# robotic-vision-lab/CropNeRF-A-Neural-Radiance-Field-Based-Framework

Measured on AMD Instinct MI355X. Metric: ray_samples_per_sec, higher is better.
Workload: dtype f32 (matrix products: bf16 hi+lo operand split, f32 accumulate); 1 GPU; plant_1-shaped synthetic scene (P-rand), 800x800, 192 samples/ray, 65536-ray batch, mode M-uniform, fused cn_render_rays, eval (no jitter); rays_per_batch=65536, samples_per_ray=192, mode=uniform, matrix_precision=split_bf16 (FruitNerfModelConfig default; exact fp32: secondary.exact_fp32_ms)

## Files before the change

### cropnerf-a-neural-radiance-field-based-framework_amd/csrc/cn_common.hpp

```cpp
#pragma once

#include <hip/hip_runtime.h>

#include <cstdarg>
#include <cstdio>
#include <cstring>
#include <mutex>
#include <type_traits>

#include "../../include/cropnerf_hip.h"

#define CN_WAVE 64

namespace cn {

void set_error(const char* fmt, ...);

inline int check_launch(const char* what) {
  hipError_t e = hipGetLastError();
  if (e != hipSuccess) {
    set_error("%s: %s", what, hipGetErrorString(e));
    return CN_ERR_LAUNCH;
  }
  return CN_OK;
}

#define CN_REQUIRE(cond, code, ...) \
  do {                              \
    if (!(cond)) {                  \
      cn::set_error(__VA_ARGS__);   \
      return (code);                \
    }                               \
  } while (0)

inline hipStream_t as_stream(cn_stream_t s) { return reinterpret_cast<hipStream_t>(s); }

// ... 35 lines not shown
#define CN_P2 805459861u

struct Lvl {
  unsigned off, mask, m1, m2;
  float scale;
};

struct GridDev {
  const void* table;
  int num_levels;
  int half;
  float pos_offset;
  unsigned off[CN_MAX_LEVELS], mask[CN_MAX_LEVELS], m1[CN_MAX_LEVELS], m2[CN_MAX_LEVELS];
  float scale[CN_MAX_LEVELS];
  __host__ __device__ __forceinline__ Lvl level(int l) const {
    Lvl v;
    v.off = off[l];
    v.mask = mask[l];
    v.m1 = m1[l];
    v.m2 = m2[l];
    v.scale = scale[l];
    return v;
  }
  __host__ __device__ __forceinline__ const float* table_f32() const { return static_cast<const float*>(table); }
};

inline GridDev make_grid_dev(const cn_grid& g) {
  GridDev d;
  d.table = g.table;
  d.num_levels = g.num_levels;
  d.half = g.table_dtype == CN_TABLE_F16;
  d.pos_offset = g.layout == CN_GRID_TCNN ? 0.5f : 0.f;
  const unsigned T = 1u << g.log2_table_size;
  for (int i = 0; i < CN_MAX_LEVELS; ++i) {
    const bool live = i < g.num_levels;
    d.scale[i] = live ? g.scalings[i] : 0.f;
    const int b = (live && g.layout == CN_GRID_TCNN) ? g.level_bits[i] : 0;
    d.off[i] = !live ? 0u : (g.layout == CN_GRID_TCNN ? g.level_offset[i] : (unsigned)i * T);
    d.m1[i] = b ? 1u << b : CN_P1;
    d.m2[i] = b ? 1u << (2 * b) : CN_P2;
    d.mask[i] = b ? (1u << (3 * b)) - 1u : T - 1u;
  }
  return d;
}

inline int check_grid(const cn_grid& g, bool need_f32, const char* who) {
  CN_REQUIRE(g.table, CN_ERR_INVALID, "%s: null hash table", who);
  CN_REQUIRE(g.num_levels >= 1 && g.num_levels <= CN_MAX_LEVELS, CN_ERR_UNSUPPORTED, "%s: %d grid levels", who,
             g.num_levels);
  CN_REQUIRE(g.layout == CN_GRID_TORCH || g.layout == CN_GRID_TCNN, CN_ERR_INVALID, "%s: grid layout %d", who, g.layout);
  CN_REQUIRE(g.table_dtype == CN_TABLE_F32 || g.table_dtype == CN_TABLE_F16, CN_ERR_INVALID, "%s: table dtype %d", who,
             g.table_dtype);
  CN_REQUIRE(!need_f32 || g.table_dtype == CN_TABLE_F32, CN_ERR_UNSUPPORTED,
             "%s: needs an fp32 hash table (half tables are inference-only)", who);
  CN_REQUIRE(g.log2_table_size >= 1 && g.log2_table_size <= 24, CN_ERR_UNSUPPORTED, "%s: log2 table size %d", who,
             g.log2_table_size);
  unsigned long long entries = (unsigned long long)g.num_levels << g.log2_table_size;
  if (g.layout == CN_GRID_TCNN) {
    entries = 0;
    for (int l = 0; l < g.num_levels; ++l) {
      const int b = g.level_bits[l];
      CN_REQUIRE(b <= 9, CN_ERR_UNSUPPORTED, "%s: dense level %d with %d bits per axis", who, l, b);
      CN_REQUIRE(g.level_offset[l] % 2 == 0, CN_ERR_INVALID, "%s: level %d starts at the odd entry %u", who, l,
                 g.level_offset[l]);
      const unsigned long long end = (unsigned long long)g.level_offset[l] + (b ? 1ull << (3 * b) : 1ull << g.log2_table_size);
      if (end > entries) entries = end;
    }
  }
  CN_REQUIRE(entries * 8ull <= (1ull << 31), CN_ERR_UNSUPPORTED, "%s: hash table larger than 2 GiB", who);
  const uintptr_t align = g.table_dtype == CN_TABLE_F16 ? 7u : 15u;
  CN_REQUIRE((reinterpret_cast<uintptr_t>(g.table) & align) == 0, CN_ERR_INVALID,
             "%s: the hash table must be %u-byte aligned", who, (unsigned)align + 1u);
  return CN_OK;
}
// ... 61 lines not shown
      const float coef = 2.f * inv * inv * (inv - 1.f) * s;
      gx *= k;
      gy *= k;
      gz *= k;
      if (axv >= ayv && axv >= azv) gx += x < 0.f ? -coef : coef;
      else if (ayv >= azv) gy += y < 0.f ? -coef : coef;
      else gz += z < 0.f ? -coef : coef;
    }
  } else {
    gx *= sc.inv_extent[0] * sel;
    gy *= sc.inv_extent[1] * sel;
    gz *= sc.inv_extent[2] * sel;
  }
}

typedef const float __attribute__((address_space(4)))* cfloat_ptr;
__device__ __forceinline__ cfloat_ptr as_const(const float* p) { return (cfloat_ptr)(unsigned long long)p; }

template <bool HALF = false>
__device__ __forceinline__ float2 hash_gather(const void* __restrict__ table, unsigned entry) {
  if constexpr (HALF) {
    typedef _Float16 h2 __attribute__((ext_vector_type(2)));
    const h2 v = *reinterpret_cast<const h2*>(reinterpret_cast<const char*>(table) + (size_t)(entry << 2));
    return make_float2((float)v.x, (float)v.y);
  } else {
    return *reinterpret_cast<const float2*>(reinterpret_cast<const char*>(table) + (size_t)(entry << 3));
  }
}

struct Cell {
  float ox, oy, oz;
  unsigned hx0, hx1, hy0, hy1, hz0, hz1;
};
template <bool OFFSET = true>
__device__ __forceinline__ Cell hash_cell(const Lvl& lv, float pos_offset, float px, float py, float pz) {
  const float sx = OFFSET ? fmaf(px, lv.scale, pos_offset) : px * lv.scale;
  const float sy = OFFSET ? fmaf(py, lv.scale, pos_offset) : py * lv.scale;
  const float sz = OFFSET ? fmaf(pz, lv.scale, pos_offset) : pz * lv.scale;
  const float fx = floorf(sx), fy = floorf(sy), fz = floorf(sz);
  Cell c;
  c.ox = sx - fx;
  c.oy = sy - fy;
  c.oz = sz - fz;
  const unsigned ix = (unsigned)(int)fx, iy = (unsigned)(int)fy, iz = (unsigned)(int)fz;
  c.hx0 = ix;
  c.hx1 = ix + 1u;
  c.hy0 = __umul24(iy, lv.m1);
  c.hy1 = c.hy0 + lv.m1;
  c.hz0 = __umul24(iz, lv.m2);
  c.hz1 = c.hz0 + lv.m2;
  return c;
}

template <bool HALF = false>
__device__ __forceinline__ float2 hash_level(const void* __restrict__ table, const Lvl& lv, float pos_offset, float px,
                                             float py, float pz) {
  const Cell k = hash_cell(lv, pos_offset, px, py, pz);
  const float ox = k.ox, oy = k.oy, oz = k.oz;
  float2 ccc = hash_gather<HALF>(table, ((k.hx1 ^ k.hy1 ^ k.hz1) & lv.mask) + lv.off);
  float2 cfc = hash_gather<HALF>(table, ((k.hx1 ^ k.hy0 ^ k.hz1) & lv.mask) + lv.off);
  float2 ffc = hash_gather<HALF>(table, ((k.hx0 ^ k.hy0 ^ k.hz1) & lv.mask) + lv.off);
  float2 fcc = hash_gather<HALF>(table, ((k.hx0 ^ k.hy1 ^ k.hz1) & lv.mask) + lv.off);
  float2 ccf = hash_gather<HALF>(table, ((k.hx1 ^ k.hy1 ^ k.hz0) & lv.mask) + lv.off);
  float2 cff = hash_gather<HALF>(table, ((k.hx1 ^ k.hy0 ^ k.hz0) & lv.mask) + lv.off);
  float2 fff = hash_gather<HALF>(table, ((k.hx0 ^ k.hy0 ^ k.hz0) & lv.mask) + lv.off);
  float2 fcf = hash_gather<HALF>(table, ((k.hx0 ^ k.hy1 ^ k.hz0) & lv.mask) + lv.off);
  float mx = 1.f - ox, my = 1.f - oy, mz = 1.f - oz;
  typedef float v2f __attribute__((ext_vector_type(2)));
  auto V = [](float2 t) {
    v2f v;
    v.x = t.x;
    v.y = t.y;
    return v;
  };
  const v2f f03 = V(ccc) * ox + V(fcc) * mx, f12 = V(cfc) * ox + V(ffc) * mx;
  const v2f f56 = V(cff) * ox + V(fff) * mx, f47 = V(ccf) * ox + V(fcf) * mx;
  const v2f a = f03 * oy + f12 * my, b = f47 * oy + f56 * my;
// ... 17 lines not shown
  float2 ccf = hash_gather<HALF>(table, ((k.hx1 ^ k.hy1 ^ k.hz0) & lv.mask) + lv.off);
  float2 cff = hash_gather<HALF>(table, ((k.hx1 ^ k.hy0 ^ k.hz0) & lv.mask) + lv.off);
  float2 fff = hash_gather<HALF>(table, ((k.hx0 ^ k.hy0 ^ k.hz0) & lv.mask) + lv.off);
  float2 fcf = hash_gather<HALF>(table, ((k.hx0 ^ k.hy1 ^ k.hz0) & lv.mask) + lv.off);
  const float mx = 1.f - ox, my = 1.f - oy, mz = 1.f - oz;
  auto V = [](float2 t) {
    v2f_t v;
    v.x = t.x;
    v.y = t.y;
    return v;
  };
  const v2f_t f03 = V(ccc) * ox + V(fcc) * mx, f12 = V(cfc) * ox + V(ffc) * mx;
  const v2f_t f56 = V(cff) * ox + V(fff) * mx, f47 = V(ccf) * ox + V(fcf) * mx;
  const v2f_t a = f03 * oy + f12 * my, b = f47 * oy + f56 * my;
  const v2f_t rv = a * oz + b * mz;
  const v2f_t d03 = V(ccc) - V(fcc), d12 = V(cfc) - V(ffc), d56 = V(cff) - V(fff), d47 = V(ccf) - V(fcf);
  jx = ((d03 * oy + d12 * my) * oz + (d47 * oy + d56 * my) * mz) * lv.scale;
  jy = ((f03 - f12) * oz + (f47 - f56) * mz) * lv.scale;
  jz = (a - b) * lv.scale;
  float2 r;
  r.x = rv.x;
  r.y = rv.y;
  return r;
}

template <bool HALF>
struct XpLoads {
  typedef float f4 __attribute__((ext_vector_type(4)));
  typedef _Float16 h4 __attribute__((ext_vector_type(4)));
  typedef _Float16 h2 __attribute__((ext_vector_type(2)));
  typename std::conditional<HALF, h4, f4>::type pr[4];
  typename std::conditional<HALF, h2, float2>::type up[4];
  unsigned bits;
  float ox, oy, oz;
};
template <bool HALF = false>
__device__ __forceinline__ XpLoads<HALF> hash_level_xpair_issue(const void* __restrict__ table, const Lvl& lv, float pos_offset,
                                                                float px, float py, float pz) {
  const Cell k = hash_cell(lv, pos_offset, px, py, pz);
  const char* base = reinterpret_cast<const char*>(table);
  const unsigned pair_mask = lv.mask & ~1u;
  const unsigned hyz[4] = {k.hy0 ^ k.hz0, k.hy1 ^ k.hz0, k.hy0 ^ k.hz1, k.hy1 ^ k.hz1};
  const bool odd = (k.hx0 & 1u) != 0u;
  XpLoads<HALF> L;
  L.bits = odd ? 16u : 0u;
  L.ox = k.ox;
  L.oy = k.oy;
  L.oz = k.oz;
#pragma unroll
  for (int r = 0; r < 4; ++r) {
    const unsigned x = k.hx0 ^ hyz[r];
    L.bits |= (x & 1u) << r;
    const unsigned e = (x & pair_mask) + lv.off;
    if constexpr (HALF) L.pr[r] = *reinterpret_cast<const typename XpLoads<HALF>::h4*>(base + (size_t)(e << 2));
    else L.pr[r] = *reinterpret_cast<const typename XpLoads<HALF>::f4*>(base + (size_t)(e << 3));
  }
#pragma unroll
  for (int r = 0; r < 4; ++r) {
    if constexpr (HALF) L.up[r] = typename XpLoads<HALF>::h2{(_Float16)0.f, (_Float16)0.f};
    else L.up[r] = make_float2(0.f, 0.f);
  }
  if (odd) {
#pragma unroll
    for (int r = 0; r < 4; ++r) {
      const unsigned e = ((k.hx1 ^ hyz[r]) & lv.mask) + lv.off;
      if constexpr (HALF) L.up[r] = *reinterpret_cast<const typename XpLoads<HALF>::h2*>(base + (size_t)(e << 2));
      else L.up[r] = *reinterpret_cast<const float2*>(base + (size_t)(e << 3));
    }
  }
  return L;
}
template <bool HALF = false>
__device__ __forceinline__ float2 hash_level_xpair_blend(const XpLoads<HALF>& L) {
  const bool odd = (L.bits & 16u) != 0u;
  typedef float v2f __attribute__((ext_vector_type(2)));
  const float ox = L.ox, oy = L.oy, oz = L.oz;
  const float mx = 1.f - ox, my = 1.f - oy, mz = 1.f - oz;
  const float oxe = odd ? 0.f : ox;
  v2f row[4];
#pragma unroll
  for (int r = 0; r < 4; ++r) {
    const bool second = ((L.bits >> r) & 1u) != 0u;
    const float wa = second ? oxe : mx, wb = second ? mx : oxe;
    v2f a, b, u;
    a.x = (float)L.pr[r].x;
    a.y = (float)L.pr[r].y;
    b.x = (float)L.pr[r].z;
    b.y = (float)L.pr[r].w;
    u.x = (float)L.up[r].x;
    u.y = (float)L.up[r].y;
    row[r] = u * ox + (b * wb + a * wa);
  }
  const v2f a2 = row[3] * oy + row[2] * my, b2 = row[1] * oy + row[0] * my;
  const v2f rv = a2 * oz + b2 * mz;
  float2 r;
  r.x = rv.x;
  r.y = rv.y;
  asm volatile("" : "+v"(r.x), "+v"(r.y));
  return r;
}
template <bool HALF = false>
__device__ __forceinline__ float2 hash_level_xpair(const void* __restrict__ table, const Lvl& lv, float pos_offset, float px,
                                                   float py, float pz) {
  return hash_level_xpair_blend<HALF>(hash_level_xpair_issue<HALF>(table, lv, pos_offset, px, py, pz));
}

__device__ __forceinline__ Lvl lane_level(const GridDev& g, int l) {
  Lvl v = g.level(0);
#pragma unroll
  for (int k = 1; k < CN_MAX_LEVELS; ++k) {
    const Lvl w = g.level(k);
    v.off = l == k ? w.off : v.off;
    v.mask = l == k ? w.mask : v.mask;
    v.m1 = l == k ? w.m1 : v.m1;
    v.m2 = l == k ? w.m2 : v.m2;
    v.scale = l == k ? w.scale : v.scale;
  }
  return v;
}

constexpr int LVL_REC_FLOATS = 16 + 64;
__device__ __forceinline__ void lds_level_fill(float* rec, const GridDev& g, int tid) {
  if (tid < CN_MAX_LEVELS) {
    const Lvl v = lane_level(g, tid);
// ... 29 lines not shown
  const Cell k = hash_cell<OFFSET>(lv, pos_offset, px, py, pz);
  const float ox = k.ox, oy = k.oy, oz = k.oz;
  float2 ccc = hash_gather<HALF>(table, ((k.hx1 ^ k.hy1 ^ k.hz1) & lv.mask) + lv.off);
  float2 cfc = hash_gather<HALF>(table, ((k.hx1 ^ k.hy0 ^ k.hz1) & lv.mask) + lv.off);
  float2 ffc = hash_gather<HALF>(table, ((k.hx0 ^ k.hy0 ^ k.hz1) & lv.mask) + lv.off);
  float2 fcc = hash_gather<HALF>(table, ((k.hx0 ^ k.hy1 ^ k.hz1) & lv.mask) + lv.off);
  float2 ccf = hash_gather<HALF>(table, ((k.hx1 ^ k.hy1 ^ k.hz0) & lv.mask) + lv.off);
  float2 cff = hash_gather<HALF>(table, ((k.hx1 ^ k.hy0 ^ k.hz0) & lv.mask) + lv.off);
  float2 fff = hash_gather<HALF>(table, ((k.hx0 ^ k.hy0 ^ k.hz0) & lv.mask) + lv.off);
  float2 fcf = hash_gather<HALF>(table, ((k.hx0 ^ k.hy1 ^ k.hz0) & lv.mask) + lv.off);
  float mx = 1.f - ox, my = 1.f - oy, mz = 1.f - oz;
  float2 r;
  {
    float f03 = ccc.x * ox + fcc.x * mx, f12 = cfc.x * ox + ffc.x * mx;
    float f56 = cff.x * ox + fff.x * mx, f47 = ccf.x * ox + fcf.x * mx;
    float a = f03 * oy + f12 * my, b = f47 * oy + f56 * my;
    r.x = a * oz + b * mz;
  }
  {
    float f03 = ccc.y * ox + fcc.y * mx, f12 = cfc.y * ox + ffc.y * mx;
    float f56 = cff.y * ox + fff.y * mx, f47 = ccf.y * ox + fcf.y * mx;
    float a = f03 * oy + f12 * my, b = f47 * oy + f56 * my;
    r.y = a * oz + b * mz;
  }
  return r;
}

typedef _Float16 f16x2 __attribute__((ext_vector_type(2)));
typedef unsigned u32x2p __attribute__((ext_vector_type(2)));
struct PkLoads {
  u32x2p pr[4];
  unsigned up[4];
  unsigned bits;
  unsigned wxy, wzz;
};
template <bool OFFSET = true>
__device__ __forceinline__ PkLoads hash_level_pk_issue(const void* __restrict__ table, const Lvl& lv, float pos_offset, float px,
                                                       float py, float pz) {
  const Cell k = hash_cell<OFFSET>(lv, pos_offset, px, py, pz);
  const char* base = reinterpret_cast<const char*>(table);
  const unsigned pair_mask = lv.mask & ~1u;
  const unsigned hyz[4] = {k.hy0 ^ k.hz0, k.hy1 ^ k.hz0, k.hy0 ^ k.hz1, k.hy1 ^ k.hz1};
  PkLoads L;
  {
    const _Float16 hx = (_Float16)k.ox, hy = (_Float16)k.oy, hz = (_Float16)k.oz;
    const f16x2 xy = {hx, hy}, zz = {hz, hz};
    L.wxy = __builtin_bit_cast(unsigned, xy);
    L.wzz = __builtin_bit_cast(unsigned, zz);
  }
  const bool odd = (k.hx0 & 1u) != 0u;
  L.bits = odd ? 16u : 0u;
#pragma unroll
  for (int r = 0; r < 4; ++r) {
    const unsigned x = k.hx0 ^ hyz[r];
    L.bits |= (x & 1u) << r;
    L.pr[r] = *reinterpret_cast<const u32x2p*>(base + (size_t)(((x & pair_mask) + lv.off) << 2));
    L.up[r] = 0u;
  }
#if !defined(CN_ABLATE_X1)
  if (odd) {
#pragma unroll
    for (int r = 0; r < 4; ++r) {
      L.up[r] = *reinterpret_cast<const unsigned*>(base + (size_t)((((k.hx1 ^ hyz[r]) & lv.mask) + lv.off) << 2));
    }
  }
#endif
  return L;
}
__device__ __forceinline__ unsigned hash_level_pk_blend(const PkLoads& L) {
  const bool odd = (L.bits & 16u) != 0u;
  f16x2 lo[4], hi[4];
#pragma unroll
  for (int r = 0; r < 4; ++r) {
    const bool second = (L.bits & (1u << r)) != 0u;
    const unsigned a = L.pr[r].x, b = L.pr[r].y;
    lo[r] = __builtin_bit_cast(f16x2, second ? b : a);
    const unsigned upv = L.up[r];
    hi[r] = __builtin_bit_cast(f16x2, odd ? upv : (second ? a : b));
  }
  const f16x2 wxy = __builtin_bit_cast(f16x2, L.wxy), wz = __builtin_bit_cast(f16x2, L.wzz);
  const f16x2 wx = {wxy.x, wxy.x}, wy = {wxy.y, wxy.y};
  const f16x2 xff = lo[0] + (hi[0] - lo[0]) * wx, xcf = lo[1] + (hi[1] - lo[1]) * wx;
  const f16x2 xfc = lo[2] + (hi[2] - lo[2]) * wx, xcc = lo[3] + (hi[3] - lo[3]) * wx;
  const f16x2 yf = xff + (xcf - xff) * wy, yc = xfc + (xcc - xfc) * wy;
  const f16x2 r = yf + (yc - yf) * wz;
  return __builtin_bit_cast(unsigned, r);
}
__device__ __forceinline__ unsigned pk_pin(unsigned v) {
  asm volatile("" : "+v"(v));
  return v;
}
template <bool OFFSET = true>
__device__ __forceinline__ unsigned hash_level_pk(const void* __restrict__ table, const Lvl& lv, float pos_offset, float px,
                                                  float py, float pz) {
  return hash_level_pk_blend(hash_level_pk_issue<OFFSET>(table, lv, pos_offset, px, py, pz));
}


__device__ __forceinline__ float linspace01(int i, int steps) {
  float step = 1.f / (float)(steps - 1);
  int half = steps / 2;
  return i < half ? step * (float)i : 1.f - step * (float)(steps - i - 1);
}

__device__ __forceinline__ float spacing_fn(int mode, float x) {
  if (mode == CN_SPACING_PIECEWISE) return x < 1.f ? x / 2.f : 1.f - 1.f / (2.f * x);
  return x;
}
__device__ __forceinline__ float spacing_fn_inv(int mode, float x) {
  if (mode == CN_SPACING_PIECEWISE) return x < 0.5f ? 2.f * x : 1.f / (2.f - 2.f * x);
  return x;
}
__device__ __forceinline__ float spacing_to_euclid(int mode, float x, float s_near, float s_far) {
  return spacing_fn_inv(mode, x * s_far + (1.f - x) * s_near);
}

__device__ __forceinline__ void sh_deg4(float x, float y, float z, float* c) {
  float xx = x * x, yy = y * y, zz = z * z;
  c[0] = 0.28209479177387814f;
  c[1] = 0.4886025119029199f * y;
  c[2] = 0.4886025119029199f * z;
  c[3] = 0.4886025119029199f * x;
  c[4] = 1.0925484305920792f * x * y;
  c[5] = 1.0925484305920792f * y * z;
  c[6] = 0.9461746957575601f * zz - 0.31539156525251999f;
  c[7] = 1.0925484305920792f * x * z;
  c[8] = 0.5462742152960396f * (xx - yy);
  c[9] = 0.5900435899266435f * y * (3.f * xx - yy);
  c[10] = 2.890611442640554f * x * y * z;
  c[11] = 0.4570457994644658f * y * (5.f * zz - 1.f);
  c[12] = 0.3731763325901154f * z * (5.f * zz - 3.f);
  c[13] = 0.4570457994644658f * x * (5.f * zz - 1.f);
  c[14] = 1.445305721320277f * z * (xx - yy);
  c[15] = 0.5900435899266435f * x * (xx - 3.f * yy);
}

// ... 9 lines not shown
```

### cropnerf-a-neural-radiance-field-based-framework_amd/csrc/render_f16.hpp

```cpp
#pragma once

namespace cn {

#ifndef CN_F16_WAVES_PER_SIMD
#define CN_F16_WAVES_PER_SIMD 4
#endif
#ifndef CN_F16_LEVELS_IN_FLIGHT
#define CN_F16_LEVELS_IN_FLIGHT 2
#endif

constexpr int F16_IMG_FLOATS = BF16_BLOCKS * 256;
constexpr int F16_TAIL_FLOATS = BLOB_FLOATS - OFF_B0;
constexpr int F16_LDS_FLOATS = F16_IMG_FLOATS + F16_TAIL_FLOATS + FUSED_WAVES * WAVE_SCRATCH;
static_assert(F16_IMG_FLOATS % 4 == 0 && F16_TAIL_FLOATS % 4 == 0 && OFF_B0 % 4 == 0, "copied as float4");
#define CN_F16_T(OFF) (F16_IMG_FLOATS + (OFF) - OFF_B0)

template <bool HALF, bool GENERIC>
__global__ void __launch_bounds__(FUSED_THREADS, CN_F16_WAVES_PER_SIMD) render_f16_kernel(FusedArgs A) {
  __shared__ __align__(16) float lds[F16_LDS_FLOATS];
  {
    const float4* src = reinterpret_cast<const float4*>(A.blob);
    float4* dst = reinterpret_cast<float4*>(lds);
    for (int i = threadIdx.x; i < F16_IMG_FLOATS / 4; i += FUSED_THREADS) dst[i] = src[i];
    for (int i = threadIdx.x; i < F16_TAIL_FLOATS / 4; i += FUSED_THREADS) dst[F16_IMG_FLOATS / 4 + i] = src[OFF_B0 / 4 + i];
// ... 7 lines not shown

  const int nchunks = (S + 63) >> 6;
  const int xcd = blockIdx.x & 7;
  const int slot = blockIdx.x >> 3;
  const long long stride = (long long)(gridDim.x >> 3) * FUSED_WAVES;
  const bool striped = A.image_width > 0;
  const long long per_xcd = (A.num_rays + 7) >> 3;
  const int nstripe = 8 * A.stripes_per_xcd;
  const int cw = striped ? (A.image_width + nstripe - 1) / nstripe : 0;
  const long long first_row = striped ? A.pixel_start / A.image_width : 0;
  const long long last_row = striped ? (A.pixel_start + A.num_rays - 1) / A.image_width : 0;
  const long long rows = last_row - first_row + 1;
  const long long items = striped ? rows * cw * A.stripes_per_xcd : min(per_xcd, max(A.num_rays - xcd * per_xcd, 0LL));

  for (long long q = slot * FUSED_WAVES + wave; q < items; q += stride) {
    long long rr;
    if (striped) {
      const long long sq = q / (rows * cw);
      const long long qq = q - sq * rows * cw;
      const long long vrow = qq / cw;
      const int col = (int)(sq * 8 + xcd) * cw + (int)(qq - vrow * cw);
      rr = (first_row + vrow) * A.image_width + col - A.pixel_start;
      if (col >= A.image_width || rr < 0 || rr >= A.num_rays) continue;
    } else {
      rr = xcd * per_xcd + q;
    }
    const long long r = __builtin_amdgcn_readfirstlane((int)rr);
    const float ox = A.origins[3 * r], oy = A.origins[3 * r + 1], oz = A.origins[3 * r + 2];
    const float dx = A.directions[3 * r], dy = A.directions[3 * r + 1], dz = A.directions[3 * r + 2];
    const float sn = spacing_fn(A.spacing, A.nears[r]), sf = spacing_fn(A.spacing, A.fars[r]);
    const float* bins = A.bins ? A.bins + r * (long long)(S + 1) : nullptr;
    auto edge = [&](int i) -> float {
      i = min(i, S);
      return bins ? bins[i] : spacing_to_euclid(A.spacing, linspace01(i, S + 1), sn, sf);
    };

    CompositeState st;
    for (int ch = 0; ch < nchunks; ++ch) {
      const int c0 = ch * 64;
      const float e_lo = edge(c0 + lane);
      const float e_top = edge(c0 + 64);
      __builtin_amdgcn_wave_barrier();
      tbuf[lane] = e_lo;
      if (lane == 0) tbuf[64] = e_top;
      __builtin_amdgcn_fence(__ATOMIC_RELEASE, "wavefront");
      __builtin_amdgcn_wave_barrier();

      float my_dlogit = 0.f, my_sel = 0.f;
#pragma unroll 1
      for (int half = 0; half < 2; ++half) {
        float px[2], py[2], pz[2];
        bool sel[2];
#pragma unroll
        for (int c = 0; c < 2; ++c) {
          const int k = 32 * half + 16 * c + j;
          const float mid = (tbuf[k] + tbuf[k + 1]) / 2.f;
          px[c] = ox + dx * mid;
          py[c] = oy + dy * mid;
          pz[c] = oz + dz * mid;
          sel[c] = normalize_position(A.scene, px[c], py[c], pz[c]);
        }
        u32x4v featp[2];
        {
          const f32x4 lvl_scale = *reinterpret_cast<const f32x4*>(lds + CN_F16_T(OFF_SCALE) + 4 * g);
          const float pos_off = GENERIC ? A.grid.pos_offset : 0.f;
          if constexpr (HALF && !CN_ABLATE_GATHER) {
            PkLoads cur = hash_level_pk_issue<GENERIC>(
// ... 96 lines not shown
```

### cropnerf-a-neural-radiance-field-based-framework_amd/csrc/render_fused.hip

```cpp
#include "composite_dev.hpp"

namespace cn {

typedef float f32x4 __attribute__((ext_vector_type(4)));

constexpr int OFF_A0 = 0;
constexpr int OFF_A1 = 2048;
constexpr int OFF_AS0 = 3072;
constexpr int OFF_AC0 = 4096;
constexpr int OFF_AC1 = 5120;
constexpr int OFF_B0 = 9216;
constexpr int OFF_B1 = 9280;
constexpr int OFF_BS0 = 9296;
constexpr int OFF_BC1 = 9360;
constexpr int OFF_WF = 9424;
constexpr int OFF_WRGB = 9488;
constexpr int OFF_MISC = 9680;
constexpr int OFF_WSH = 9688;
constexpr int OFF_SCALE = 10712;
constexpr int OFF_LVL = 10728;
constexpr int BLOB_FLOATS = 10728 + 64;
static_assert(BLOB_FLOATS % 4 == 0, "blob is copied as float4");
static_assert(OFF_A0 == 0 && OFF_B0 == 18 * 512, "the split-bf16 images reuse the fp32 A-operand region block for block");
constexpr int WAVE_SCRATCH = 200;
// ... 165 lines not shown
        const unsigned w = f == 0 ? p.grid.off[k] : (f == 1 ? p.grid.mask[k] : (f == 2 ? p.grid.m1[k] : p.grid.m2[k]));
        u = q == k ? w : u;
      }
      v = __builtin_bit_cast(float, u);
    } else {
      int q = i - BLOB_FLOATS;
      int row = q >> 6, n = q & 63;
      v = p.bc0[n];
      if (p.app_mode != CN_APP_ZEROS) {
        const float* a = p.app_mode == CN_APP_PER_CAMERA ? p.emb + row * 32 : p.emb_mean;
        for (int k = 0; k < 32; ++k) v = fmaf(R16(p.wc0[n * 63 + 31 + k]), R16(a[k]), v);
      }
      app_bias[q] = v;
      continue;
    }
    blob[i] = v;
  }
}

struct FusedArgs {
  GridDev grid;
  SceneDev scene;
  const float* blob;
  const float* blob_ext;
  const float* app_bias;
  const float* origins;
  const float* directions;
  const float* nears;
  const float* fars;
  const int64_t* cam_idx;
  const float* bins;
  long long num_rays;
  int S;
  int spacing;
  int bg_mode;
  float bg[3];
  int app_per_camera;
  int sh_unit;
  int eval_clamp;
  float early_stop;
  int image_width;
  int stripes_per_xcd;
  long long pixel_start;
  float *out_rgb, *out_acc, *out_depth, *out_sem, *out_cmap, *out_w;
  float *s_density, *s_rgb, *s_sem, *s_pos;
  int64_t* s_label;
};

#if CN_ABLATE_MLP
#define MFMA(a, b, c) ((c) + (a) * (b))
#else
#define MFMA(a, b, c) __builtin_amdgcn_mfma_f32_16x16x4f32((a), (b), (c), 0, 0, 0)
#endif

__device__ __forceinline__ float relu1(float x) {
  int i = __builtin_bit_cast(int, x);
  return __builtin_bit_cast(float, i > 0 ? i : 0);
}
__device__ __forceinline__ f32x4 relu4(f32x4 v) {
  f32x4 r;
  r.x = relu1(v.x);
  r.y = relu1(v.y);
  r.z = relu1(v.z);
  r.w = relu1(v.w);
  return r;
}
// ... 50 lines not shown
  const int xcd = blockIdx.x & 7;
  const int slot = blockIdx.x >> 3;
  const long long stride = (long long)(gridDim.x >> 3) * FUSED_WAVES;
  const bool striped = A.image_width > 0;
  const long long per_xcd = (A.num_rays + 7) >> 3;
  const int nstripe = 8 * A.stripes_per_xcd;
  const int cw = striped ? (A.image_width + nstripe - 1) / nstripe : 0;
  const long long first_row = striped ? A.pixel_start / A.image_width : 0;
  const long long last_row = striped ? (A.pixel_start + A.num_rays - 1) / A.image_width : 0;
  const long long rows = last_row - first_row + 1;
  const long long items =
      striped ? rows * cw * A.stripes_per_xcd : min(per_xcd, max(A.num_rays - xcd * per_xcd, 0LL));

  for (long long q = slot * FUSED_WAVES + wave; q < items; q += stride) {
    long long rr;
    if (striped) {
      const long long sq = q / (rows * cw);
      const long long qq = q - sq * rows * cw;
      const long long vrow = qq / cw;
      const int col = (int)(sq * 8 + xcd) * cw + (int)(qq - vrow * cw);
      rr = (first_row + vrow) * A.image_width + col - A.pixel_start;
      if (col >= A.image_width || rr < 0 || rr >= A.num_rays) continue;
    } else {
      rr = xcd * per_xcd + q;
    }
    const long long r = __builtin_amdgcn_readfirstlane((int)rr);
    const float ox = A.origins[3 * r], oy = A.origins[3 * r + 1], oz = A.origins[3 * r + 2];
    const float dx = A.directions[3 * r], dy = A.directions[3 * r + 1], dz = A.directions[3 * r + 2];
    const float near = A.nears[r], far = A.fars[r];
    const float sn = spacing_fn(A.spacing, near), sf = spacing_fn(A.spacing, far);
    const float* bins = A.bins ? A.bins + r * (long long)(S + 1) : nullptr;
    auto edge = [&](int i) -> float {
      i = min(i, S);
      return bins ? bins[i] : spacing_to_euclid(A.spacing, linspace01(i, S + 1), sn, sf);
    };

    if (!DENSITY_ONLY) {
      float sx = dx, sy = dy, sz = dz;
      if (!A.sh_unit) {
        sx = (dx + 1.f) / 2.f;
        sy = (dy + 1.f) / 2.f;
        sz = (dz + 1.f) / 2.f;
      }
      float sh[16];
      sh_deg4(sx, sy, sz, sh);
      long long row = A.app_per_camera ? A.cam_idx[r] : 0;
      float bias = A.app_bias[row * 64 + lane];
      const f32x4* wsh = reinterpret_cast<const f32x4*>(lds + OFF_WSH + lane * 16);
#pragma unroll
      for (int q = 0; q < 4; ++q) {
        f32x4 w = wsh[q];
        bias = fmaf(w.x, sh[4 * q + 0], bias);
        bias = fmaf(w.y, sh[4 * q + 1], bias);
        bias = fmaf(w.z, sh[4 * q + 2], bias);
        bias = fmaf(w.w, sh[4 * q + 3], bias);
      }
      __builtin_amdgcn_wave_barrier();
      scratch[lane] = bias;
      __builtin_amdgcn_fence(__ATOMIC_RELEASE, "wavefront");
      __builtin_amdgcn_wave_barrier();
    }

    CompositeState st;
    for (int c0 = 0; c0 < S; c0 += 64) {
      const float e_lo = edge(c0 + lane);
      const float e_top = edge(c0 + 64);
      __builtin_amdgcn_wave_barrier();
// ... 376 lines not shown
  P.wh = params->sem_head_weight;
  P.bh = params->sem_head_bias;
  P.wc0 = params->color.weight[0];
  P.bc0 = params->color.bias[0];
  P.wc1 = params->color.weight[1];
  P.bc1 = params->color.bias[1];
  P.wc2 = params->color.weight[2];
  P.bc2 = params->color.bias[2];
  P.emb = params->appearance;
  P.num_images = params->num_images;
  P.app_mode = opts->app_mode;
  P.app_rows = opts->app_mode == CN_APP_PER_CAMERA ? params->num_images : 1;
  float* emb_mean = app_bias + (size_t)(params->num_images > 0 ? params->num_images : 1) * 64;
  P.emb_mean = emb_mean;
  if (opts->app_mode == CN_APP_MEAN)
    hipLaunchKernelGGL(prep_mean_kernel, dim3(1), dim3(256), 0, s, params->appearance, params->num_images, emb_mean);
  P.grid = A.grid;
  hipLaunchKernelGGL(prep_kernel, dim3(48), dim3(256), 0, s, P, blob, app_bias);
  rc = check_launch("cn_render prep");
  if (rc) return rc;

  A.scene = make_scene_dev(*scene);
  A.blob = blob;
  A.blob_ext = P.ext;
  A.app_bias = app_bias;
  A.origins = origins;
  A.directions = directions;
  A.nears = nears;
  A.fars = fars;
  A.cam_idx = cam_idx;
  A.bins = bins;
  A.num_rays = num_rays;
  A.S = opts->num_samples;
  A.spacing = opts->spacing;
  A.bg_mode = opts->bg_mode;
  A.bg[0] = opts->bg_color[0];
  A.bg[1] = opts->bg_color[1];
  A.bg[2] = opts->bg_color[2];
  A.app_per_camera = opts->app_mode == CN_APP_PER_CAMERA;
  A.sh_unit = opts->sh_unit_dir;
  A.eval_clamp = opts->eval_clamp;
  A.early_stop = early_stop;
  A.image_width = opts->image_width > 0 ? opts->image_width : 0;
  A.stripes_per_xcd = A.image_width > 0 ? (A.image_width + 96) / 192 : 1;
  if (A.stripes_per_xcd < 1) A.stripes_per_xcd = 1;
  A.pixel_start = opts->pixel_start;
  const long long cap = f16_density ? dev->res_f16_density
                                    : (PER_SAMPLE ? dev->res_sample : (opts->density_only ? dev->res_density : dev->res_full));
  const long long want = (((num_rays + FUSED_WAVES - 1) / FUSED_WAVES) + 7) / 8 * 8;
  const unsigned blocks = (unsigned)(want < cap ? want : cap);
  if (split_blocks) {
    const size_t lds_bytes = bf16 ? SPLIT_LDS_BYTES_BF16 : SPLIT_LDS_BYTES;
    const char* pack_env = getenv("CN_SPLIT_PACK");
    const bool pack = mm == MM_FP32 && opts->num_samples > 32 && opts->num_samples <= 48 && early_stop == 0.f &&
                      !(pack_env && atoi(pack_env) == 0);
#define CN_SPLIT_LAUNCH(MM, H)                                                                                       \
  do {                                                                                                               \
    if (generic)                                                                                                     \
      hipLaunchKernelGGL((render_split_kernel<PER_SAMPLE, MM, H, true>), dim3(split_blocks), dim3(SPLIT_THREADS),    \
                         lds_bytes, s, A);                                                                           \
    else                                                                                                             \
      hipLaunchKernelGGL((render_split_kernel<PER_SAMPLE, MM, H, false>), dim3(split_blocks), dim3(SPLIT_THREADS),   \
                         lds_bytes, s, A);                                                                           \
  } while (0)
    if (mm == MM_F16 && half) CN_SPLIT_LAUNCH(MM_F16, true);
    else if (mm == MM_F16) CN_SPLIT_LAUNCH(MM_F16, false);
// ... 78 lines not shown
```

### cropnerf-a-neural-radiance-field-based-framework_amd/csrc/render_split.hpp

```cpp
#pragma once

namespace cn {

#ifndef CN_SPLIT_LEVELS_IN_FLIGHT
#define CN_SPLIT_LEVELS_IN_FLIGHT 4
#endif
#ifndef CN_TEAM_RAYS
#define CN_TEAM_RAYS 4
#endif
#ifndef CN_TEAM_RAYS_PS
#define CN_TEAM_RAYS_PS 1
#endif
#ifndef CN_SPLIT_G
#define CN_SPLIT_G 8
#endif
#ifndef CN_SPLIT_MPG
#define CN_SPLIT_MPG 1
#endif
constexpr int SPLIT_G = CN_SPLIT_G, SPLIT_MPG = CN_SPLIT_MPG;
constexpr int SPLIT_PAIRS = SPLIT_G * SPLIT_MPG;
constexpr int SPLIT_THREADS = (SPLIT_G + SPLIT_PAIRS) * 64;
static_assert(SPLIT_THREADS <= 1024, "at most 16 waves per workgroup");
constexpr int XCH_FLOATS = 16 * 64 + 64;
constexpr int PAIR_SCRATCH = 2 * XCH_FLOATS + 64 + 68 + 68 + 4;
constexpr int PAIR_FLAGS = 2 * XCH_FLOATS + 64 + 68 + 68;
constexpr size_t SPLIT_LDS_BYTES = (size_t)(BLOB_FLOATS + SPLIT_PAIRS * PAIR_SCRATCH) * sizeof(float);
constexpr size_t SPLIT_LDS_BYTES_BF16 = SPLIT_LDS_BYTES + (size_t)BF16_EXT_FLOATS * sizeof(float);
constexpr int PACK_SCRATCH = 64 + 68 + 68;
constexpr size_t SPLIT_LDS_BYTES_PACK = SPLIT_LDS_BYTES + (size_t)(SPLIT_PAIRS * PACK_SCRATCH) * sizeof(float);

typedef __bf16 bf16x8 __attribute__((ext_vector_type(8)));

__device__ __forceinline__ void split_bf16(const f32x4& a, const f32x4& b, bf16x8& hi, bf16x8& lo) {
#pragma unroll
  for (int j = 0; j < 8; ++j) {
    const float x = j < 4 ? a[j] : b[j - 4];
    const __bf16 h = (__bf16)x;
    hi[j] = h;
    lo[j] = (__bf16)(x - (float)h);
  }
}
__device__ __forceinline__ f32x4 mfma_split(const bf16x8& ah, const bf16x8& al, const bf16x8& bh, const bf16x8& bl, f32x4 acc) {
  acc = __builtin_amdgcn_mfma_f32_16x16x32_bf16(ah, bh, acc, 0, 0, 0);
  acc = __builtin_amdgcn_mfma_f32_16x16x32_bf16(ah, bl, acc, 0, 0, 0);
  acc = __builtin_amdgcn_mfma_f32_16x16x32_bf16(al, bh, acc, 0, 0, 0);
  return acc;
}

__device__ __forceinline__ bf16x8 split_bf16_k16(const f32x4& a) {
  bf16x8 r;
#pragma unroll
  for (int j = 0; j < 4; ++j) {
    const __bf16 h = (__bf16)a[j];
    r[j] = h;
    r[4 + j] = (__bf16)(a[j] - (float)h);
  }
  return r;
}
__device__ __forceinline__ f32x4 mfma_split_k16(const bf16x8& ah, const bf16x8& al, const bf16x8& b, f32x4 acc) {
  acc = __builtin_amdgcn_mfma_f32_16x16x32_bf16(ah, b, acc, 0, 0, 0);
  acc = __builtin_amdgcn_mfma_f32_16x16x32_bf16(al, b, acc, 0, 0, 0);
  return acc;
}

typedef _Float16 f16x8 __attribute__((ext_vector_type(8)));
typedef unsigned u32x4v __attribute__((ext_vector_type(4)));
__device__ __forceinline__ f16x8 cvt_f16x8(const f32x4& a, const f32x4& b) {
  f16x8 r;
#pragma unroll
  for (int j = 0; j < 4; ++j) {
    r[j] = (_Float16)a[j];
    r[4 + j] = (_Float16)b[j];
  }
  return r;
}
__device__ __forceinline__ f32x4 mfma_f16(const f16x8& a, const f16x8& b, f32x4 acc) {
  return __builtin_amdgcn_mfma_f32_16x16x32_f16(a, b, acc, 0, 0, 0);
}

struct SplitRay {
  float ox, oy, oz, dx, dy, dz, sn, sf;
  const float* bins;
  long long r;
  int chunk;
  bool valid;
};

struct QuadSched {
  int cw, wq, span, ns1, nh, nodd, t0, qlo, nq, llo;
};
// ... 43 lines not shown
        rr = l < P.nh ? l : (l < P.nh + P.nodd ? P.nh + (l - P.nh) * W + W - 1 : P.t0 + (l - P.nh - P.nodd));
      }
    } else {
    const long long sq = q / (rows * cw);
    const long long qq = q - sq * rows * cw;
    const long long vrow = qq / cw;
    const int col = (int)(sq * 8 + xcd) * cw + (int)(qq - vrow * cw);
    rr = (first_row + vrow) * A.image_width + col - A.pixel_start;
    if (col >= A.image_width || rr < 0 || rr >= A.num_rays) return;
    }
  } else {
    rr = xcd * per_xcd + q;
  }
  if (chunks_per_ray > 0) {
    ray.chunk = (int)(rr / A.num_rays);
    rr -= (long long)ray.chunk * A.num_rays;
  }
  const long long r = __builtin_amdgcn_readfirstlane((int)rr);
  ray.r = r;
  ray.ox = A.origins[3 * r];
  ray.oy = A.origins[3 * r + 1];
  ray.oz = A.origins[3 * r + 2];
  ray.dx = A.directions[3 * r];
  ray.dy = A.directions[3 * r + 1];
  ray.dz = A.directions[3 * r + 2];
  ray.sn = spacing_fn(A.spacing, A.nears[r]);
  ray.sf = spacing_fn(A.spacing, A.fars[r]);
  ray.bins = A.bins ? A.bins + r * (long long)(A.S + 1) : nullptr;
  ray.valid = true;
}

__device__ __forceinline__ float split_edge(const FusedArgs& A, const SplitRay& ray, int i) {
  i = min(i, A.S);
  return ray.bins ? ray.bins[i] : spacing_to_euclid(A.spacing, linspace01(i, A.S + 1), ray.sn, ray.sf);
}

__device__ __forceinline__ void split_fill_edges(const FusedArgs& A, const SplitRay& ray, int c0, float* tb, int lane) {
  const float e_lo = split_edge(A, ray, c0 + lane);
  const float e_top = split_edge(A, ray, c0 + 64);
  __builtin_amdgcn_wave_barrier();
  tb[lane] = e_lo;
  if (lane == 0) tb[64] = e_top;
  __builtin_amdgcn_fence(__ATOMIC_RELEASE, "wavefront");
  __builtin_amdgcn_wave_barrier();
}

template <bool PER_SAMPLE, int MM = MM_FP32, bool HALF = false, bool GENERIC = false, bool PACK = false>
__global__ void __launch_bounds__(SPLIT_THREADS) render_split_kernel(FusedArgs A) {
  static_assert(!PACK || MM == MM_FP32, "the packed schedule exists for the exact-fp32 kernel (the other modes gather in teams)");
  constexpr bool BF16 = MM == MM_BF16, F16 = MM == MM_F16;
  constexpr int TR = PER_SAMPLE ? CN_TEAM_RAYS_PS : CN_TEAM_RAYS;
  constexpr bool TEAM = !PACK && MM != MM_FP32 && TR > 1 && (SPLIT_MPG == 1) && (SPLIT_G % TR == 0) && !CN_ABLATE_GATHER;
  constexpr bool QUAD = TEAM && TR == 4;
  extern __shared__ __align__(16) float lds[];
  constexpr int OFF_EXT = BLOB_FLOATS + SPLIT_PAIRS * PAIR_SCRATCH;
  {
    const float4* src = reinterpret_cast<const float4*>(A.blob);
    float4* dst = reinterpret_cast<float4*>(lds);
    for (int i = threadIdx.x; i < BLOB_FLOATS / 4; i += SPLIT_THREADS) dst[i] = src[i];
    if constexpr (BF16) {
      const float4* esrc = reinterpret_cast<const float4*>(A.blob_ext);
      float4* edst = reinterpret_cast<float4*>(lds + OFF_EXT);
      for (int i = threadIdx.x; i < BF16_EXT_FLOATS / 4; i += SPLIT_THREADS) edst[i] = esrc[i];
    }
    if (threadIdx.x < SPLIT_PAIRS * 4)
      reinterpret_cast<int*>(lds + BLOB_FLOATS + (threadIdx.x >> 2) * PAIR_SCRATCH + PAIR_FLAGS)[threadIdx.x & 3] =
          (threadIdx.x & 3) == 2 ? -1 : 0;
// ... 70 lines not shown
                const unsigned long long bp = reinterpret_cast<unsigned long long>(tr.bins);
                w[0] = tr.ox; w[1] = tr.oy; w[2] = tr.oz; w[3] = tr.dx;
                w[4] = tr.dy; w[5] = tr.dz; w[6] = tr.sn; w[7] = tr.sf;
                reinterpret_cast<unsigned*>(w)[8] = (unsigned)bp;
                reinterpret_cast<unsigned*>(w)[9] = (unsigned)(bp >> 32);
                reinterpret_cast<int*>(w)[10] = tr.chunk;
                reinterpret_cast<int*>(w)[11] = tr.valid ? 1 : 0;
              }
            }
            __builtin_amdgcn_fence(__ATOMIC_RELEASE, "wavefront");
            __builtin_amdgcn_wave_barrier();
          }
          float* ring0 = lds + BLOB_FLOATS + pair0 * PAIR_SCRATCH;
          const int mcol = lane & 15, rsel = mcol & (TR - 1), sidx = mcol / TR;
          bool any = false, active = false;
#pragma unroll
          for (int t = 0; t < TR; ++t) {
            const bool a = reinterpret_cast<const int*>(trec + 16 * t)[11] != 0 &&
                           !(!PER_SAMPLE && A.early_stop > 0.f &&
                             reinterpret_cast<volatile int*>(ring0 + t * PAIR_SCRATCH + PAIR_FLAGS)[2] == (int)qi);
            any = any || a;
            active = rsel == t ? a : active;
          }
          if (any) {
            if (active) {
              const f32x4 ra = *reinterpret_cast<const f32x4*>(trec + 16 * rsel);
              const f32x4 rb = *reinterpret_cast<const f32x4*>(trec + 16 * rsel + 4);
              const u32x4v rc = *reinterpret_cast<const u32x4v*>(trec + 16 * rsel + 8);
              const float rox = ra.x, roy = ra.y, roz = ra.z, rdx = ra.w, rdy = rb.x, rdz = rb.y, rsn = rb.z, rsf = rb.w;
              const float* rbins = reinterpret_cast<const float*>((unsigned long long)rc.x | ((unsigned long long)rc.y << 32));
              const int chunk = PER_SAMPLE ? (int)rc.z : (k >> 1), half = k & 1;
              auto edge = [&](int i) -> float {
                i = min(i, S);
                return rbins ? rbins[i] : spacing_to_euclid(A.spacing, linspace01(i, S + 1), rsn, rsf);
              };
              float px[2], py[2], pz[2];
              bool sel[2];
              int col[2];
#pragma unroll
              for (int h = 0; h < 2; ++h) {
                col[h] = SPW * sub + (SPW / 2) * h + sidx;
                const int i0 = chunk * 64 + 32 * half + col[h];
                const float mid = (edge(i0) + edge(i0 + 1)) / 2.f;
                px[h] = rox + rdx * mid;
                py[h] = roy + rdy * mid;
                pz[h] = roz + rdz * mid;
                sel[h] = normalize_position(A.scene, px[h], py[h], pz[h]);
              }
              u32x4v featp[2];
              f32x4 feat[2][2];
              const f32x4 lvl_scale = *reinterpret_cast<const f32x4*>(lds + OFF_SCALE + 4 * g);
              const float pos_off = GENERIC ? A.grid.pos_offset : 0.f;
              if constexpr (F16 && HALF) {
                PkLoads cur = hash_level_pk_issue<GENERIC>(A.grid.table, lane_level_rec<GENERIC>(lds + OFF_LVL, A.grid, 4 * g, lvl_scale[0]),
                                                           pos_off, px[0], py[0], pz[0]);
#pragma unroll
                for (int u = 0; u < 8; ++u) {
                  PkLoads nxt;
                  if (u < 7) {
                    const int qn = (u + 1) >> 1, hn = (u + 1) & 1;
                    nxt = hash_level_pk_issue<GENERIC>(A.grid.table,
                                                       lane_level_rec<GENERIC>(lds + OFF_LVL, A.grid, 4 * g + qn, lvl_scale[qn]), pos_off,
                                                       px[hn], py[hn], pz[hn]);
                  }
                  featp[u & 1][u >> 1] = pk_pin(hash_level_pk_blend(cur));
                  if (u < 7) cur = nxt;
                }
// ... 543 lines not shown
```

Measured before the change: 7.802 billion samples/s.

## Trim hash-grid and bf16-split ALU work: fract-based cells, parity bits, packed split, precomputed linspace step

Several independent ALU reductions in the hot render kernel. For non-negative offset coordinates, hash cells now use the hardware fract instruction and a truncating int conversion instead of floorf. The per-row parity bits of the x-pair blend are derived from one bit plus a level-wide flip, relying on the hash primes sharing parity. The bf16 hi/lo split now converts pairs with packed vector conversions, and the linspace reciprocal is computed once on the host. Empty asm barriers pin blend operands in registers. Truncation equals floor only when coordinates are non-negative, which is assumed rather than checked for the TCNN +0.5 offset path.

```diff
diff --git a/cropnerf-a-neural-radiance-field-based-framework_amd/csrc/cn_common.hpp b/cropnerf-a-neural-radiance-field-based-framework_amd/csrc/cn_common.hpp
--- a/cropnerf-a-neural-radiance-field-based-framework_amd/csrc/cn_common.hpp
+++ b/cropnerf-a-neural-radiance-field-based-framework_amd/csrc/cn_common.hpp
@@ -2,6 +2,7 @@
 
 #include <hip/hip_runtime.h>
 
+#include <cassert>
 #include <cstdarg>
 #include <cstdio>
 #include <cstring>
@@ -103,6 +104,7 @@
   d.half = g.table_dtype == CN_TABLE_F16;
   d.pos_offset = g.layout == CN_GRID_TCNN ? 0.5f : 0.f;
   const unsigned T = 1u << g.log2_table_size;
+  static_assert(((CN_P1 ^ CN_P2) & 1u) == 0u, "the hash primes share their parity");
   for (int i = 0; i < CN_MAX_LEVELS; ++i) {
     const bool live = i < g.num_levels;
     d.scale[i] = live ? g.scalings[i] : 0.f;
@@ -111,6 +113,7 @@
     d.m1[i] = b ? 1u << b : CN_P1;
     d.m2[i] = b ? 1u << (2 * b) : CN_P2;
     d.mask[i] = b ? (1u << (3 * b)) - 1u : T - 1u;
+    assert(((d.m1[i] ^ d.m2[i]) & 1u) == 0u);
   }
   return d;
 }
@@ -238,17 +241,26 @@
   float ox, oy, oz;
   unsigned hx0, hx1, hy0, hy1, hz0, hz1;
 };
-template <bool OFFSET = true>
+template <bool OFFSET = true, bool NONNEG = false>
 __device__ __forceinline__ Cell hash_cell(const Lvl& lv, float pos_offset, float px, float py, float pz) {
+  static_assert(OFFSET || !NONNEG, "the floor-free form needs the explicit fmaf of OFFSET");
   const float sx = OFFSET ? fmaf(px, lv.scale, pos_offset) : px * lv.scale;
   const float sy = OFFSET ? fmaf(py, lv.scale, pos_offset) : py * lv.scale;
   const float sz = OFFSET ? fmaf(pz, lv.scale, pos_offset) : pz * lv.scale;
-  const float fx = floorf(sx), fy = floorf(sy), fz = floorf(sz);
   Cell c;
-  c.ox = sx - fx;
-  c.oy = sy - fy;
-  c.oz = sz - fz;
-  const unsigned ix = (unsigned)(int)fx, iy = (unsigned)(int)fy, iz = (unsigned)(int)fz;
+  unsigned ix, iy, iz;
+  if constexpr (NONNEG) {
+    c.ox = __builtin_amdgcn_fractf(sx);
+    c.oy = __builtin_amdgcn_fractf(sy);
+    c.oz = __builtin_amdgcn_fractf(sz);
+    ix = (unsigned)(int)sx, iy = (unsigned)(int)sy, iz = (unsigned)(int)sz;
+  } else {
+    const float fx = floorf(sx), fy = floorf(sy), fz = floorf(sz);
+    c.ox = sx - fx;
+    c.oy = sy - fy;
+    c.oz = sz - fz;
+    ix = (unsigned)(int)fx, iy = (unsigned)(int)fy, iz = (unsigned)(int)fz;
+  }
   c.hx0 = ix;
   c.hx1 = ix + 1u;
   c.hy0 = __umul24(iy, lv.m1);
@@ -332,25 +344,26 @@
   typename std::conditional<HALF, h4, f4>::type pr[4];
   typename std::conditional<HALF, h2, float2>::type up[4];
   unsigned bits;
+  unsigned flip;
   float ox, oy, oz;
 };
 template <bool HALF = false>
 __device__ __forceinline__ XpLoads<HALF> hash_level_xpair_issue(const void* __restrict__ table, const Lvl& lv, float pos_offset,
                                                                 float px, float py, float pz) {
-  const Cell k = hash_cell(lv, pos_offset, px, py, pz);
+  const Cell k = hash_cell<true, true>(lv, pos_offset, px, py, pz);
   const char* base = reinterpret_cast<const char*>(table);
   const unsigned pair_mask = lv.mask & ~1u;
   const unsigned hyz[4] = {k.hy0 ^ k.hz0, k.hy1 ^ k.hz0, k.hy0 ^ k.hz1, k.hy1 ^ k.hz1};
   const bool odd = (k.hx0 & 1u) != 0u;
   XpLoads<HALF> L;
-  L.bits = odd ? 16u : 0u;
+  L.bits = (odd ? 16u : 0u) | ((k.hx0 ^ hyz[0]) & 1u);
+  L.flip = lv.m1 & 1u;
   L.ox = k.ox;
   L.oy = k.oy;
   L.oz = k.oz;
 #pragma unroll
   for (int r = 0; r < 4; ++r) {
     const unsigned x = k.hx0 ^ hyz[r];
-    L.bits |= (x & 1u) << r;
     const unsigned e = (x & pair_mask) + lv.off;
     if constexpr (HALF) L.pr[r] = *reinterpret_cast<const typename XpLoads<HALF>::h4*>(base + (size_t)(e << 2));
     else L.pr[r] = *reinterpret_cast<const typename XpLoads<HALF>::f4*>(base + (size_t)(e << 3));
@@ -377,11 +390,13 @@
   const float ox = L.ox, oy = L.oy, oz = L.oz;
   const float mx = 1.f - ox, my = 1.f - oy, mz = 1.f - oz;
   const float oxe = odd ? 0.f : ox;
+  const bool second0 = (L.bits & 1u) != 0u, flip = L.flip != 0u;
+  const float wa0 = second0 ? oxe : mx, wb0 = second0 ? mx : oxe;
+  const float wa1 = flip ? wb0 : wa0, wb1 = flip ? wa0 : wb0;
   v2f row[4];
 #pragma unroll
   for (int r = 0; r < 4; ++r) {
-    const bool second = ((L.bits >> r) & 1u) != 0u;
-    const float wa = second ? oxe : mx, wb = second ? mx : oxe;
+    const float wa = (r == 1 || r == 2) ? wa1 : wa0, wb = (r == 1 || r == 2) ? wb1 : wb0;
     v2f a, b, u;
     a.x = (float)L.pr[r].x;
     a.y = (float)L.pr[r].y;
@@ -389,7 +404,9 @@
     b.y = (float)L.pr[r].w;
     u.x = (float)L.up[r].x;
     u.y = (float)L.up[r].y;
+    asm volatile("" : "+v"(a), "+v"(b), "+v"(u));
     row[r] = u * ox + (b * wb + a * wa);
+    asm volatile("" : "+v"(row[r]));
   }
   const v2f a2 = row[3] * oy + row[2] * my, b2 = row[1] * oy + row[0] * my;
   const v2f rv = a2 * oz + b2 * mz;
@@ -485,12 +502,13 @@
   u32x2p pr[4];
   unsigned up[4];
   unsigned bits;
+  unsigned flip;
   unsigned wxy, wzz;
 };
 template <bool OFFSET = true>
 __device__ __forceinline__ PkLoads hash_level_pk_issue(const void* __restrict__ table, const Lvl& lv, float pos_offset, float px,
                                                        float py, float pz) {
-  const Cell k = hash_cell<OFFSET>(lv, pos_offset, px, py, pz);
+  const Cell k = hash_cell<OFFSET, OFFSET>(lv, pos_offset, px, py, pz);
   const char* base = reinterpret_cast<const char*>(table);
   const unsigned pair_mask = lv.mask & ~1u;
   const unsigned hyz[4] = {k.hy0 ^ k.hz0, k.hy1 ^ k.hz0, k.hy0 ^ k.hz1, k.hy1 ^ k.hz1};
@@ -502,11 +520,11 @@
     L.wzz = __builtin_bit_cast(unsigned, zz);
   }
   const bool odd = (k.hx0 & 1u) != 0u;
-  L.bits = odd ? 16u : 0u;
+  L.bits = (odd ? 16u : 0u) | ((k.hx0 ^ hyz[0]) & 1u);
+  L.flip = lv.m1 & 1u;
 #pragma unroll
   for (int r = 0; r < 4; ++r) {
     const unsigned x = k.hx0 ^ hyz[r];
-    L.bits |= (x & 1u) << r;
     L.pr[r] = *reinterpret_cast<const u32x2p*>(base + (size_t)(((x & pair_mask) + lv.off) << 2));
     L.up[r] = 0u;
   }
@@ -523,9 +541,10 @@
 __device__ __forceinline__ unsigned hash_level_pk_blend(const PkLoads& L) {
   const bool odd = (L.bits & 16u) != 0u;
   f16x2 lo[4], hi[4];
+  const bool second0 = (L.bits & 1u) != 0u, second1 = ((L.bits ^ L.flip) & 1u) != 0u;
 #pragma unroll
   for (int r = 0; r < 4; ++r) {
-    const bool second = (L.bits & (1u << r)) != 0u;
+    const bool second = (r == 1 || r == 2) ? second1 : second0;
     const unsigned a = L.pr[r].x, b = L.pr[r].y;
     lo[r] = __builtin_bit_cast(f16x2, second ? b : a);
     const unsigned upv = L.up[r];
@@ -550,11 +569,12 @@
 }
 
 
-__device__ __forceinline__ float linspace01(int i, int steps) {
-  float step = 1.f / (float)(steps - 1);
+inline float linspace_step(int steps) { return 1.f / (float)(steps - 1); }
+__device__ __forceinline__ float linspace01(int i, int steps, float step) {
   int half = steps / 2;
   return i < half ? step * (float)i : 1.f - step * (float)(steps - i - 1);
 }
+__device__ __forceinline__ float linspace01(int i, int steps) { return linspace01(i, steps, 1.f / (float)(steps - 1)); }
 
 __device__ __forceinline__ float spacing_fn(int mode, float x) {
   if (mode == CN_SPACING_PIECEWISE) return x < 1.f ? x / 2.f : 1.f - 1.f / (2.f * x);
diff --git a/cropnerf-a-neural-radiance-field-based-framework_amd/csrc/render_f16.hpp b/cropnerf-a-neural-radiance-field-based-framework_amd/csrc/render_f16.hpp
--- a/cropnerf-a-neural-radiance-field-based-framework_amd/csrc/render_f16.hpp
+++ b/cropnerf-a-neural-radiance-field-based-framework_amd/csrc/render_f16.hpp
@@ -63,7 +63,7 @@
     const float* bins = A.bins ? A.bins + r * (long long)(S + 1) : nullptr;
     auto edge = [&](int i) -> float {
       i = min(i, S);
-      return bins ? bins[i] : spacing_to_euclid(A.spacing, linspace01(i, S + 1), sn, sf);
+      return bins ? bins[i] : spacing_to_euclid(A.spacing, linspace01(i, S + 1, A.lin_step), sn, sf);
     };
 
     CompositeState st;
diff --git a/cropnerf-a-neural-radiance-field-based-framework_amd/csrc/render_fused.hip b/cropnerf-a-neural-radiance-field-based-framework_amd/csrc/render_fused.hip
--- a/cropnerf-a-neural-radiance-field-based-framework_amd/csrc/render_fused.hip
+++ b/cropnerf-a-neural-radiance-field-based-framework_amd/csrc/render_fused.hip
@@ -221,6 +221,7 @@
   const float* bins;
   long long num_rays;
   int S;
+  float lin_step;
   int spacing;
   int bg_mode;
   float bg[3];
@@ -337,7 +338,7 @@
     const float* bins = A.bins ? A.bins + r * (long long)(S + 1) : nullptr;
     auto edge = [&](int i) -> float {
       i = min(i, S);
-      return bins ? bins[i] : spacing_to_euclid(A.spacing, linspace01(i, S + 1), sn, sf);
+      return bins ? bins[i] : spacing_to_euclid(A.spacing, linspace01(i, S + 1, A.lin_step), sn, sf);
     };
 
     if (!DENSITY_ONLY) {
@@ -780,6 +781,7 @@
   A.bins = bins;
   A.num_rays = num_rays;
   A.S = opts->num_samples;
+  A.lin_step = linspace_step(opts->num_samples + 1);
   A.spacing = opts->spacing;
   A.bg_mode = opts->bg_mode;
   A.bg[0] = opts->bg_color[0];
diff --git a/cropnerf-a-neural-radiance-field-based-framework_amd/csrc/render_split.hpp b/cropnerf-a-neural-radiance-field-based-framework_amd/csrc/render_split.hpp
--- a/cropnerf-a-neural-radiance-field-based-framework_amd/csrc/render_split.hpp
+++ b/cropnerf-a-neural-radiance-field-based-framework_amd/csrc/render_split.hpp
@@ -31,14 +31,24 @@
 
 typedef __bf16 bf16x8 __attribute__((ext_vector_type(8)));
 
+typedef float f32x2s __attribute__((ext_vector_type(2)));
+typedef __bf16 bf16x2s __attribute__((ext_vector_type(2)));
+typedef unsigned u32x4s __attribute__((ext_vector_type(4)));
+__device__ __forceinline__ void split_bf16_pair(float x0, float x1, unsigned& hi, unsigned& lo) {
+  const f32x2s x = {x0, x1};
+  const unsigned h = __builtin_bit_cast(unsigned, __builtin_convertvector(x, bf16x2s));
+  const f32x2s hf = {__builtin_bit_cast(float, h << 16), __builtin_bit_cast(float, h & 0xffff0000u)};
+  hi = h;
+  lo = __builtin_bit_cast(unsigned, __builtin_convertvector(x - hf, bf16x2s));
+}
 __device__ __forceinline__ void split_bf16(const f32x4& a, const f32x4& b, bf16x8& hi, bf16x8& lo) {
-#pragma unroll
-  for (int j = 0; j < 8; ++j) {
-    const float x = j < 4 ? a[j] : b[j - 4];
-    const __bf16 h = (__bf16)x;
-    hi[j] = h;
-    lo[j] = (__bf16)(x - (float)h);
-  }
+  unsigned h[4], l[4];
+  split_bf16_pair(a.x, a.y, h[0], l[0]);
+  split_bf16_pair(a.z, a.w, h[1], l[1]);
+  split_bf16_pair(b.x, b.y, h[2], l[2]);
+  split_bf16_pair(b.z, b.w, h[3], l[3]);
+  hi = __builtin_bit_cast(bf16x8, u32x4s{h[0], h[1], h[2], h[3]});
+  lo = __builtin_bit_cast(bf16x8, u32x4s{l[0], l[1], l[2], l[3]});
 }
 __device__ __forceinline__ f32x4 mfma_split(const bf16x8& ah, const bf16x8& al, const bf16x8& bh, const bf16x8& bl, f32x4 acc) {
   acc = __builtin_amdgcn_mfma_f32_16x16x32_bf16(ah, bh, acc, 0, 0, 0);
@@ -48,14 +58,10 @@
 }
 
 __device__ __forceinline__ bf16x8 split_bf16_k16(const f32x4& a) {
-  bf16x8 r;
-#pragma unroll
-  for (int j = 0; j < 4; ++j) {
-    const __bf16 h = (__bf16)a[j];
-    r[j] = h;
-    r[4 + j] = (__bf16)(a[j] - (float)h);
-  }
-  return r;
+  unsigned h[2], l[2];
+  split_bf16_pair(a.x, a.y, h[0], l[0]);
+  split_bf16_pair(a.z, a.w, h[1], l[1]);
+  return __builtin_bit_cast(bf16x8, u32x4s{h[0], h[1], l[0], l[1]});
 }
 __device__ __forceinline__ f32x4 mfma_split_k16(const bf16x8& ah, const bf16x8& al, const bf16x8& b, f32x4 acc) {
   acc = __builtin_amdgcn_mfma_f32_16x16x32_bf16(ah, b, acc, 0, 0, 0);
@@ -165,7 +171,7 @@
 
 __device__ __forceinline__ float split_edge(const FusedArgs& A, const SplitRay& ray, int i) {
   i = min(i, A.S);
-  return ray.bins ? ray.bins[i] : spacing_to_euclid(A.spacing, linspace01(i, A.S + 1), ray.sn, ray.sf);
+  return ray.bins ? ray.bins[i] : spacing_to_euclid(A.spacing, linspace01(i, A.S + 1, A.lin_step), ray.sn, ray.sf);
 }
 
 __device__ __forceinline__ void split_fill_edges(const FusedArgs& A, const SplitRay& ray, int c0, float* tb, int lane) {
@@ -302,7 +308,7 @@
               const int chunk = PER_SAMPLE ? (int)rc.z : (k >> 1), half = k & 1;
               auto edge = [&](int i) -> float {
                 i = min(i, S);
-                return rbins ? rbins[i] : spacing_to_euclid(A.spacing, linspace01(i, S + 1), rsn, rsf);
+                return rbins ? rbins[i] : spacing_to_euclid(A.spacing, linspace01(i, S + 1, A.lin_step), rsn, rsf);
               };
               float px[2], py[2], pz[2];
               bool sel[2];
```

Measured after the change: 8.096 billion samples/s (median of 6 runs). +3.8%, better.
